# mrluin/TextualDegRemoval

Measured on AMD Instinct MI355X. Metric: train images/sec (512x512, bs=4/GPU), higher is better.
Workload: dtype f32 (3xbf16-split MFMA: 24-bit operand significands on the full fp32 exponent range, fp32 accumulate; unscaled gradients, no loss scale, no step-skip guard; tensors fp32 -- the MASA-encoder ResidualBlock activations / gradients as three bf16 planes whose sum IS the fp32 value, bit for bit)

## Files before the change

### include/tdr.h

```cpp
#ifndef TDR_H
#define TDR_H
#include <stdint.h>
#ifdef __cplusplus
extern "C" {
#endif

#define TDR_ABI_VERSION 112
int tdr_version(void);
const char* tdr_last_error(void);

typedef struct TdrStepGuard {
    float scale, inv_scale, max_scale;
    int good, growth_interval;
    int step, skipped, finite;
    float bc1, bc2_sqrt;
} TdrStepGuard;

typedef struct TdrConvDesc {
    int N, Cin, H, W;
    int Cout, OH, OW;
    int KH, stride, dil, pad;
    const float* in;  int64_t in_ns;
    int gate;
    const float* kscale; int64_t kscale_ns;
    const void* wp;  int64_t wp_ns;  int Mpad;
    int wp_fmt;
    float* out; int64_t out_ns;
    int epi;
    const float* bias;  int64_t bias_ns;
    const float* scale; int64_t scale_ns;
    const float* bias2; int64_t bias2_ns; float bias2_mul;
    const float* res;   int64_t res_ns;
    const float* mask;  int64_t mask_ns;
    const float* aux;   int64_t aux_ns;
    int relu;
} TdrConvDesc;

int tdr_conv_forward(const TdrConvDesc* d, void* stream);

int tdr_conv_ck(int KH_eff);
int64_t tdr_packed_weight_floats(int M, int Kch, int KH_eff);
int tdr_pack_weights(const float* w, int Cout, int Cin, int KH, int mode, float* wp, void* stream);
int64_t tdr_packed_weight_bytes_bx3(int M, int Kch, int KH_eff);
int tdr_pack_weights_bx3(const float* w, int Cout, int Cin, int KH, int mode, void* wp, void* stream);
int tdr_pack_weights_bx3_batch(const float* w, int64_t w_stride, int B, int Cout, int Cin, int KH, int mode, void* wp,
                               void* stream);
int64_t tdr_packed_weight_bytes_hx2(int M, int Kch, int KH_eff);
int tdr_pack_weights_hx2(const float* w, int Cout, int Cin, int KH, int mode, void* wp, void* stream);
int tdr_conv_force_cfg(int kh, int cfg);
typedef struct TdrPackJob {
    const float* w; void* wp;
    int Cout, Cin, KH, mode, fmt;
    int M, Kch, KHe, CK, Mx;
    int64_t total;
    int64_t first_block;
} TdrPackJob;
int tdr_pack_job_init(TdrPackJob* job, const float* w, int Cout, int Cin, int KH, int mode, int fmt, void* wp);
int tdr_pack_weights_multi(const TdrPackJob* jobs_dev, int n_jobs, int64_t total_blocks, void* stream);
int tdr_pack_patches(const float* blk, int B, int G, int C, int BH, int BW, int PH, int PW, int pstep, int dil,
                     int off, float* wp, void* stream);

typedef struct TdrConvP16Desc {
    int N, Cin, H, W, Cout;
    const void* in;
    const void* wp; int Mpad; int wp_fmt;
    const float* bias;
    const float* res32;  int64_t res32_ns;
    const void*  res16;
    const float* mask32; int64_t mask32_ns;
    const void*  mask16;
    int relu;
    float* out32; int64_t out32_ns;
    void*  out16;
} TdrConvP16Desc;
int64_t tdr_p16_bytes(int N, int C, int H, int W);
int tdr_p16_from_f32(const float* src, int64_t src_ns, int N, int C, int H, int W, void* dst, void* stream);
int tdr_p16_to_f32(const void* src, int N, int C, int H, int W, float* dst, int64_t dst_ns, void* stream);
int64_t tdr_p16_bytes_fmt(int N, int C, int H, int W, int fmt);
int tdr_p16_from_f32_fmt(const float* src, int64_t src_ns, int N, int C, int H, int W, void* dst, int fmt, void* stream);
int tdr_p16_to_f32_fmt(const void* src, int N, int C, int H, int W, float* dst, int64_t dst_ns, int fmt, void* stream);
int tdr_conv3x3_p16(const TdrConvP16Desc* d, void* stream);
int tdr_conv3x3_p16_force_cfg(int cfg);
// ... 458 lines not shown
```

### profiles/probe_conv1x1_deep.py

```python
import os, sys
sys.path.insert(0, os.path.dirname(os.path.dirname(os.path.abspath(__file__))))
import torch
from textualdegremoval_amd import kernels as K, _lib
K.set_math('bx3')
torch.manual_seed(0)
lib = _lib.load()


def t(N, Cin, Cout, H, mode):
    xs = [torch.randn(N, Cin, H, H, device='cuda') for _ in range(2)]
    w = torch.randn(Cout, Cin, 1, 1, device='cuda') * 0.05
    wp, mp, *_ = K.pack_weights(w, mode)
    co = Cout if mode == K.PACK_FWD else Cin
    xin = xs if mode == K.PACK_FWD else [torch.randn(N, Cout, H, H, device='cuda') for _ in range(2)]
    outs = [torch.empty(N, co, H, H, device='cuda') for _ in range(2)]
    line = f'1x1 {Cin}->{Cout} @{H} N{N} {"fwd  " if mode == K.PACK_FWD else "dgrad"}:'
    flop = 2.0 * N * Cin * Cout * H * H
    for cfg in (0, 1, 2, 3, 4, 5):
        lib.tdr_conv_force_cfg(1, cfg)
        f = lambda i: K.conv_forward(xin[i & 1], wp, mp, co, 1, pad=0, out=outs[i & 1])
        for i in range(3): f(i)
        torch.cuda.synchronize()
        g = torch.cuda.CUDAGraph()
        s = torch.cuda.Stream()
        with torch.cuda.stream(s):
            with torch.cuda.graph(g, stream=s):
                for i in range(20): f(i)
        g.replay(); torch.cuda.synchronize()
        e0, e1 = torch.cuda.Event(enable_timing=True), torch.cuda.Event(enable_timing=True)
        e0.record()
        for _ in range(5): g.replay()
        e1.record(); torch.cuda.synchronize()
        us = e0.elapsed_time(e1) / 100 * 1e3
        line += f'  c{cfg} {us:6.1f} us ({flop / us * 1e-6:4.0f} TF)'
    lib.tdr_conv_force_cfg(1, 0)
    print(line, flush=True)


for (Cin, Cout) in [(1024, 2048), (1024, 1024), (1024, 512), (512, 1024), (512, 512)]:
    t(4, Cin, Cout, 32, K.PACK_FWD)
    t(4, Cin, Cout, 32, K.PACK_DGRAD_S1)
```

### textualdegremoval_amd/_lib.py

```python
import ctypes as C
import os

import torch

_HERE = os.path.dirname(os.path.abspath(__file__))
LIB_PATH = os.environ.get('TDR_LIB_PATH', os.path.join(_HERE, 'libtdr_hip.so'))

ABI_VERSION = 112
c_fp = C.c_void_p
i32, i64, f32 = C.c_int, C.c_int64, C.c_float


class TdrConvDesc(C.Structure):
    _fields_ = [
        ('N', i32), ('Cin', i32), ('H', i32), ('W', i32),
        ('Cout', i32), ('OH', i32), ('OW', i32),
        ('KH', i32), ('stride', i32), ('dil', i32), ('pad', i32),
        ('inp', c_fp), ('in_ns', i64),
        ('gate', i32),
        ('kscale', c_fp), ('kscale_ns', i64),
        ('wp', c_fp), ('wp_ns', i64), ('Mpad', i32), ('wp_fmt', i32),
        ('out', c_fp), ('out_ns', i64),
        ('epi', i32),
        ('bias', c_fp), ('bias_ns', i64),
# ... 165 lines not shown
    'tdr_dwsg_fwd': (i32, [c_fp, c_fp, c_fp, i32, i32, i32, i32, c_fp, c_fp, c_fp, c_fp]),
    'tdr_dwsg_bwd': (i32, [c_fp, c_fp, c_fp, c_fp, i32, i32, i32, i32, c_fp, c_fp, c_fp, c_fp, c_fp]),
    'tdr_dwsg_bwd_biased': (i32, [c_fp, c_fp, f32, c_fp, c_fp, c_fp, i32, i32, i32, i32, c_fp, c_fp, c_fp, c_fp, c_fp]),
    'tdr_dwsg_bwd_parts_supported': (i32, [i32]),
    'tdr_dw_param_finish': (i32, [c_fp, i32, i32, i32, i32, c_fp, c_fp, c_fp]),
    'tdr_dwgelu_fwd': (i32, [c_fp, c_fp, c_fp, i32, i32, i32, i32, c_fp, c_fp]),
    'tdr_dwgelu_bwd': (i32, [c_fp, c_fp, c_fp, c_fp, i32, i32, i32, i32, c_fp, c_fp, c_fp, c_fp, c_fp]),
    'tdr_dwconv_fwd': (i32, [c_fp, c_fp, c_fp, i32, i32, i32, i32, c_fp, c_fp]),
    'tdr_dwconv_act_fwd': (i32, [c_fp, c_fp, c_fp, i32, i32, i32, i32, i32, c_fp, c_fp]),
    'tdr_dwconv_act_bwd': (i32, [c_fp, c_fp, c_fp, c_fp, i32, i32, i32, i32, c_fp, c_fp, c_fp, c_fp, c_fp]),
    'tdr_dwpair_fwd': (i32, [c_fp, c_fp, c_fp, i32, i32, i32, i32, i32, c_fp, i64, c_fp]),
    'tdr_dwpair_bwd': (i32, [c_fp, i64, c_fp, i64, c_fp, c_fp, i32, i32, i32, i32, c_fp, c_fp, c_fp, c_fp, c_fp]),
    'tdr_dwconv_halves_fwd': (i32, [c_fp, c_fp, c_fp, i32, i32, i32, i32, i32, c_fp, c_fp, i64, c_fp]),
    'tdr_dwconv_halves_bwd': (i32, [c_fp, c_fp, i64, c_fp, c_fp, i64, c_fp, c_fp, i32, i32, i32, i32, c_fp, c_fp, c_fp, c_fp, c_fp]),
    'tdr_dwconv_bwd': (i32, [c_fp, c_fp, c_fp, i32, i32, i32, i32, c_fp, c_fp, c_fp, c_fp, c_fp]),
    'tdr_row_sumsq': (i32, [c_fp, i64, i32, i32, i32, c_fp, c_fp]),
    'tdr_mdta_pad': (i32, [i32]),
    'tdr_mdta_softmax': (i32, [c_fp, c_fp, c_fp, i32, i32, i32, c_fp, c_fp, c_fp]),
    'tdr_mdta_bwd': (i32, [c_fp, c_fp, c_fp, c_fp, c_fp, i32, i32, i32, c_fp, c_fp, c_fp, c_fp]),
    'tdr_attn_fold_proj': (i32, [c_fp, c_fp, i32, i32, i32, c_fp, c_fp]),
    'tdr_axpby_dev': (i32, [c_fp, c_fp, c_fp, i64, c_fp, c_fp]),
    'tdr_dot': (i32, [c_fp, c_fp, i64, c_fp, c_fp, c_fp]),
    'tdr_pixel_shuffle2': (i32, [c_fp, i32, i32, i32, i32, c_fp, c_fp]),
    'tdr_leaky_relu_fwd': (i32, [c_fp, i64, f32, c_fp, c_fp]),
    'tdr_leaky_relu_bwd': (i32, [c_fp, c_fp, i64, f32, c_fp, c_fp]),
    'tdr_gather_col': (i32, [c_fp, i32, i32, i32, i32, c_fp, c_fp]),
    'tdr_mapper_combine': (i32, [c_fp, c_fp, i32, i32, i32, i32, i32, i32, c_fp, c_fp]),
    'tdr_mapper_combine_bwd': (i32, [c_fp, i32, i32, i32, i32, i32, i32, c_fp, c_fp, c_fp]),
    'tdr_cross_attention_fwd': (i32, [c_fp, c_fp, c_fp, i32, i32, i32, i32, i32, i32, i32, f32, c_fp, c_fp, c_fp]),
    'tdr_cross_attention_bwd': (i32, [c_fp, c_fp, c_fp, c_fp, c_fp, c_fp, i32, i32, i32, i32, i32, i32, i32, f32, c_fp, c_fp,
                                      c_fp, c_fp, c_fp]),
    'tdr_transpose_pad': (i32, [c_fp, i32, i32, i32, i32, c_fp, c_fp]),
    'tdr_conv_force_cfg': (i32, [i32, i32]),
    'tdr_packed_weight_bytes_hx2': (i64, [i32, i32, i32]),
    'tdr_pack_weights_hx2': (i32, [c_fp, i32, i32, i32, i32, c_fp, c_fp]),
    'tdr_pack_weights_bx3_batch': (i32, [c_fp, i64, i32, i32, i32, i32, i32, c_fp, c_fp]),
    'tdr_sca_fwd': (i32, [c_fp, c_fp, c_fp, i32, i32, c_fp, c_fp]),
    'tdr_sca_bwd': (i32, [c_fp] * 8 + [i32, i32] + [c_fp] * 7 + [c_fp]),
    'tdr_gelu_fwd': (i32, [c_fp, c_fp, i32, i32, c_fp, c_fp, i64, c_fp]),
    'tdr_gelu_bwd': (i32, [c_fp, c_fp, c_fp, i64, c_fp]),
    'tdr_subsample2': (i32, [c_fp, i32, i32, i32, c_fp, c_fp]),
    'tdr_instnorm_fwd': (i32, [c_fp, c_fp, c_fp, f32, i32, i32, i32, c_fp, c_fp, c_fp, c_fp]),
    'tdr_instnorm_bwd': (i32, [c_fp] * 5 + [i32, i32, i32] + [c_fp] * 5),
    'tdr_region_affine_fwd': (i32, [c_fp, i64, c_fp, c_fp, f32, i32, i32, i32, i32, i32, c_fp, i64, c_fp, c_fp]),
    'tdr_region_affine_bwd': (i32, [c_fp, i64, c_fp, i64, c_fp, c_fp, f32, c_fp, i32, i32, i32, i32, i32, c_fp, i64, c_fp, c_fp, c_fp, c_fp]),
    'tdr_sf_dyn_vec_fwd': (i32, [C.POINTER(TdrSfDynVecDesc), c_fp]),
    'tdr_sf_dyn_vec_bwd': (i32, [C.POINTER(TdrSfDynVecBwdDesc), c_fp]),
    'tdr_sf_dynfilt_fwd': (i32, [c_fp, i64, c_fp, c_fp, c_fp, i32, i32, i32, i32, i32, i32, c_fp, c_fp, c_fp]),
    'tdr_sf_dynfilt_bwd_reduce': (i32, [c_fp, c_fp, i64, c_fp, c_fp, c_fp, i32, i32, i32, i32, i32, i32, c_fp, c_fp, c_fp, c_fp]),
    'tdr_sf_dynfilt_bwd_dx': (i32, [c_fp] * 5 + [i32] * 6 + [c_fp, i64, c_fp]),
    'tdr_convt4_weight_to_3x3': (i32, [c_fp, c_fp, i32, i32, c_fp, c_fp, c_fp]),
    'tdr_convt4_grad_from_3x3': (i32, [c_fp, c_fp, i32, i32, c_fp, c_fp, c_fp]),
    'tdr_sf_region_split': (i32, [c_fp, i64, i32, i32, i32, i32, i32, c_fp, c_fp]),
    'tdr_sf_local_affine': (i32, [c_fp, i64, c_fp, c_fp, c_fp, f32, i32, i32, i32, i32, i32, c_fp, i64, c_fp]),
    'tdr_sf_emerge': (i32, [c_fp, i64, c_fp, i32, i32, i32, c_fp, c_fp]),
    'tdr_sf_softmax_mix': (i32, [c_fp, i64, c_fp, c_fp, c_fp, i32, i32, i32, c_fp, c_fp]),
    'tdr_scaled_conv_param_grads': (i32, [c_fp] * 5 + [i32, i32] + [c_fp] * 3 + [c_fp]),
    'tdr_pair_sum_partials_multi': (i32, [c_fp, i32, i32, c_fp]),
    'tdr_dw_param_finish_nb': (i32, [i32, i32]),
    'tdr_dw_param_finish_multi': (i32, [c_fp, i32, i32, c_fp]),
    'tdr_scaled_conv_param_grads_multi': (i32, [c_fp, i32, i32, c_fp]),
    'tdr_chansum_ws_floats': (i64, [i32, i32, i32]),
    'tdr_channel_sum': (i32, [c_fp, i64, i32, i32, i32, c_fp, c_fp, c_fp]),
    'tdr_copy_rows': (i32, [c_fp, i64, c_fp, i64, i32, i64, c_fp]),
    'tdr_add_rows': (i32, [c_fp, i64, c_fp, i64, i32, i64, c_fp]),
    'tdr_pixel_unshuffle2': (i32, [c_fp, i32, i32, i32, i32, c_fp, c_fp]),
# ... 152 lines not shown
```

### textualdegremoval_amd/csrc/tdr_conv_bx3.hip

```cpp
#include <stdlib.h>
#include "tdr_common.h"
#include "tdr_conv_epi.h"
#include "tdr_pack.h"
#include "../../include/tdr.h"

typedef __bf16 bf16x8 __attribute__((ext_vector_type(8)));


namespace {

constexpr int bx_cmax(int a, int b) { return a > b ? a : b; }
constexpr int bx_plane(int NT, int TW, int KH, int S) {
    return (((NT * 32 / TW) - 1) * S + KH) * ((TW - 1) * S + KH);
}
constexpr int bx_max_plane(int NT, int KH, int S) {
    return bx_cmax(bx_plane(NT, 8, KH, S), bx_cmax(bx_plane(NT, 16, KH, S), bx_plane(NT, 32, KH, S)));
}

__device__ __forceinline__ void split3(float x, __bf16& h, __bf16& m, __bf16& l) {
    h = (__bf16)x;
    const float r = x - (float)h;
    m = (__bf16)r;
    l = (__bf16)(r - (float)m);
}
// ... 414 lines not shown
    if constexpr (EPI != EPI_PSHUF) {
        if (a.vec_epi) {
            conv_epilogue_vec<TM, TN, EPI>(a, acc, n, m0, wm, wn, oy0, ox0, lane, reinterpret_cast<float*>(smem4) + wave * (32 * 36));
            return;
        }
    }
    conv_epilogue<TM, TN, EPI>(a, acc, n, m0, wm, wn, oy0, ox0, j, kk);
}

template <int WM, int TM, int TN, int EPI, bool GATE, int SCH>
int launch_c1_hx2(const ConvArgs& a, int N, hipStream_t st) {
    constexpr int WN = 4 / WM;
    constexpr int BM = 32 * TM * WM;
    constexpr int NT = TN * WN;
    const int TW = 1 << a.tw_log2, SR = 32 >> a.tw_log2, TH = NT * SR;
    ConvArgs b = a;
    b.tiles_x = tdr_cdiv(a.OW, TW);
    const int tiles_y = tdr_cdiv(a.OH, TH);
    b.mtiles = tdr_cdiv(a.Cout, BM);
    dim3 grid(b.tiles_x * tiles_y * b.mtiles, 1, N);
    b.single_buf = 0;
    const size_t lds = 2 * 32768;
    auto kern = conv1x1_hx2_kernel<WM, TM, TN, EPI, GATE, SCH>;
    static bool attr_set = false;
    if (!attr_set) {
        (void)hipFuncSetAttribute(reinterpret_cast<const void*>(kern), hipFuncAttributeMaxDynamicSharedMemorySize, 160 * 1024);
        attr_set = true;
    }
    hipLaunchKernelGGL(kern, grid, dim3(256), lds, st, b);
    TDR_LAUNCH_CHECK("conv1x1_hx2_kernel");
    return TDR_OK;
}

inline bool c1_hx2_ok(const ConvArgs& a, int npx, int bm, int N) {
    static const bool off = tdr_tune_env("TDR_C1_OLD") != nullptr;
    static const int min_stages = tdr_tune_env("TDR_C1_STAGES") ? atoi(tdr_tune_env("TDR_C1_STAGES")) : 4;
    static const long max_blocks = tdr_tune_env("TDR_C1_BLOCKS") ? atol(tdr_tune_env("TDR_C1_BLOCKS")) : 512;
    const int ks = 8192 / npx;
    const long blocks = (long)tdr_cdiv((long)a.OH * a.OW, npx) * tdr_cdiv(a.Cout, bm) * N;
    return !off && blocks <= max_blocks && (a.Cin + ks - 1) / ks >= min_stages && a.pad == 0 && a.W % 4 == 0 && a.in_ns % 4 == 0 && (reinterpret_cast<uintptr_t>(a.in) & 15) == 0 &&
           a.H == a.OH && a.W == a.OW;
}

template <int KH, int S, int WM, int TM, int TN, int EPI, bool GATE, int SCH>
int launch_bx_cfg_s(const ConvArgs& a, int N, hipStream_t st) {
    if constexpr (KH == 1 && S == 1 && SCH != SCH_BX3 && EPI != EPI_PSHUF)
        if (c1_hx2_ok(a, 32 * TN * (4 / WM), 32 * TM * WM, N)) return launch_c1_hx2<WM, TM, TN, EPI, GATE, SCH>(a, N, st);
    constexpr int NS = SCH == SCH_BX3 ? 3 : (SCH == SCH_HX2 ? 2 : 1);
    constexpr int WN = 4 / WM;
    constexpr int BM = 32 * TM * WM;
    constexpr int NT = TN * WN;
    const int TW = 1 << a.tw_log2, SR = 32 >> a.tw_log2, TH = NT * SR;
    const int LH = (TH - 1) * S + KH, LW = (TW - 1) * S + KH;
    ConvArgs b = a;
    static const int single_env = tdr_tune_env("TDR_BX_SINGLE") ? atoi(tdr_tune_env("TDR_BX_SINGLE")) : 2;
    b.single_buf = (KH == 3 && (a.Cin + 15) / 16 <= single_env) ? 1 : 0;
    size_t lds = (size_t)(b.single_buf ? 1 : 2) * (2 * NS) * LH * LW * 16;
    if (lds < 4 * 32 * 36 * sizeof(float)) lds = 4 * 32 * 36 * sizeof(float);
    b.tiles_x = tdr_cdiv(a.OW, TW);
    const int tiles_y = tdr_cdiv(a.OH, TH);
    b.mtiles = tdr_cdiv(a.Cout, BM);
    dim3 grid(b.tiles_x * tiles_y * b.mtiles, 1, N);
    if constexpr (KH == 3 && S == 1 && SCH == SCH_HX2 && EPI == EPI_STD && !GATE) {
        static const int ring3 = tdr_tune_env("TDR_RING3") ? atoi(tdr_tune_env("TDR_RING3")) : 1;
        static const long ring_blocks3 = tdr_tune_env("TDR_RING_BLOCKS") ? atol(tdr_tune_env("TDR_RING_BLOCKS")) : 512;
        if (ring3 && ((long)grid.x * N > ring_blocks3 || TM != 1)) {
            auto kern = conv_bx3_kernel<KH, S, WM, TM, TN, EPI, GATE, SCH, 3>;
            static bool attr_set = false;
            if (!attr_set) {
                (void)hipFuncSetAttribute(reinterpret_cast<const void*>(kern), hipFuncAttributeMaxDynamicSharedMemorySize, 160 * 1024);
                attr_set = true;
            }
            hipLaunchKernelGGL(kern, grid, dim3(256), lds, st, b);
            TDR_LAUNCH_CHECK("conv_bx3_kernel(ring3)");
            return TDR_OK;
        }
    }
    if constexpr (KH == 3 && S == 1 && TM == 1 && SCH == SCH_HX2 && EPI == EPI_STD) {
        static const long ring_blocks = tdr_tune_env("TDR_RING_BLOCKS") ? atol(tdr_tune_env("TDR_RING_BLOCKS")) : 512;
        if ((long)grid.x * N <= ring_blocks) {
            auto kern = conv_bx3_kernel<KH, S, WM, TM, TN, EPI, GATE, SCH, 9>;
            static bool attr_set = false;
            if (!attr_set) {
                (void)hipFuncSetAttribute(reinterpret_cast<const void*>(kern), hipFuncAttributeMaxDynamicSharedMemorySize, 160 * 1024);
                attr_set = true;
            }
            hipLaunchKernelGGL(kern, grid, dim3(256), lds, st, b);
            TDR_LAUNCH_CHECK("conv_bx3_kernel(ring)");
            return TDR_OK;
        }
    }
    auto kern = conv_bx3_kernel<KH, S, WM, TM, TN, EPI, GATE, SCH>;
    static bool attr_set = false;
    if (!attr_set) {
        (void)hipFuncSetAttribute(reinterpret_cast<const void*>(kern), hipFuncAttributeMaxDynamicSharedMemorySize, 160 * 1024);
        attr_set = true;
    }
    hipLaunchKernelGGL(kern, grid, dim3(256), lds, st, b);
    TDR_LAUNCH_CHECK("conv_bx3_kernel");
    return TDR_OK;
}

int g_force_cfg[2] = {tdr_tune_env("TDR_BX_CFG1") ? atoi(tdr_tune_env("TDR_BX_CFG1")) : 0, tdr_tune_env("TDR_BX_CFG3") ? atoi(tdr_tune_env("TDR_BX_CFG3")) : 0};

template <int KH, int S, int WM, int TM, int TN, int EPI, bool GATE>
int launch_bx_cfg(const ConvArgs& a, int N, hipStream_t st) {
    if (a.scheme == SCH_HX2) return launch_bx_cfg_s<KH, S, WM, TM, TN, EPI, GATE, SCH_HX2>(a, N, st);
    if (a.scheme == SCH_H1) return launch_bx_cfg_s<KH, S, WM, TM, TN, EPI, GATE, SCH_H1>(a, N, st);
    return launch_bx_cfg_s<KH, S, WM, TM, TN, EPI, GATE, SCH_BX3>(a, N, st);
}

template <int KH, int S, int EPI, bool GATE>
int launch_bx_shape(const ConvArgs& a, int N, hipStream_t st) {
    const long pix = (long)a.OH * a.OW;
    auto blocks = [&](int bm, int bn) { return (long)tdr_cdiv(a.Cout, bm) * tdr_cdiv(pix, bn) * N; };
    if constexpr (S == 2) {
        if (a.Cout <= 32) return launch_bx_cfg<KH, S, 1, 1, 1, EPI, GATE>(a, N, st);
        if (a.Cout <= 64 || blocks(128, 64) < 512) return launch_bx_cfg<KH, S, 2, 1, 1, EPI, GATE>(a, N, st);
        return launch_bx_cfg<KH, S, 2, 2, 1, EPI, GATE>(a, N, st);
    } else {
        if (a.Cout <= 32) {
            if (blocks(32, 256) >= 512) return launch_bx_cfg<KH, S, 1, 1, 2, EPI, GATE>(a, N, st);
            return launch_bx_cfg<KH, S, 1, 1, 1, EPI, GATE>(a, N, st);
        }
        if (g_force_cfg[KH == 1 ? 0 : 1] == 0 && a.scheme == SCH_BX3 && a.Cin <= (KH == 1 ? 128 : 64) && blocks(64, 128) >= 2048)
            return launch_bx_cfg<KH, S, 2, 1, 2, EPI, GATE>(a, N, st);
        if constexpr (KH == 1) {
            const int force = g_force_cfg[0];
            if (force == 1) return launch_bx_cfg<KH, S, 2, 2, 2, EPI, GATE>(a, N, st);
            if (force == 2) return launch_bx_cfg<KH, S, 2, 1, 4, EPI, GATE>(a, N, st);
            if (force == 3) return launch_bx_cfg<KH, S, 2, 1, 2, EPI, GATE>(a, N, st);
            if (force == 4) return launch_bx_cfg<KH, S, 1, 1, 2, EPI, GATE>(a, N, st);
            if (force == 5) return launch_bx_cfg<KH, S, 4, 2, 2, EPI, GATE>(a, N, st);
            if (a.Cout > 64 && blocks(128, 128) >= 512) return launch_bx_cfg<KH, S, 2, 2, 2, EPI, GATE>(a, N, st);
            if (a.Cin >= 768 && a.Cout >= 256 && blocks(256, 64) >= 256 && blocks(256, 64) <= 512)
                return launch_bx_cfg<KH, S, 4, 2, 2, EPI, GATE>(a, N, st);
        } else {
            const int force3 = g_force_cfg[1];
            if (force3 == 1) return launch_bx_cfg<KH, S, 2, 2, 4, EPI, GATE>(a, N, st);
            if (force3 == 2) return launch_bx_cfg<KH, S, 2, 1, 4, EPI, GATE>(a, N, st);
            if (force3 == 3) return launch_bx_cfg<KH, S, 2, 1, 2, EPI, GATE>(a, N, st);
            if (force3 == 4) return launch_bx_cfg<KH, S, 2, 2, 2, EPI, GATE>(a, N, st);
            const bool tall_ok = blocks(128, 256) >= 1024 || a.Cout % 128 != 0 || a.scheme != SCH_HX2;
            if (a.Cout > 64 && blocks(128, 256) >= 512 && tall_ok) return launch_bx_cfg<KH, S, 2, 2, 4, EPI, GATE>(a, N, st);
        }
        if (blocks(64, 256) >= 512) return launch_bx_cfg<KH, S, 2, 1, 4, EPI, GATE>(a, N, st);
        return launch_bx_cfg<KH, S, 2, 1, 2, EPI, GATE>(a, N, st);
    }
}

__global__ void pack_weights_bx3_kernel(const float* __restrict__ w, long w_bs, int Cout, int Cin, int KH, int mode, int M,
                                        int Kch, int KHe, int MT, long total, uint4* __restrict__ wp, long wp_bs16) {
    const float* wb = w + (long)blockIdx.y * w_bs;
    uint4* ob = wp + (long)blockIdx.y * wp_bs16;
    for (long i = blockIdx.x * (long)blockDim.x + threadIdx.x; i < total; i += (long)gridDim.x * blockDim.x)
        tdr_pack_bx3_frag(wb, Cin, KH, mode, M, Kch, KHe, MT, i, ob);
}

__global__ void pack_weights_hx2_kernel(const float* __restrict__ w, int Cout, int Cin, int KH, int mode, int M, int Kch, int KHe,
                                        int MT, long total, uint4* __restrict__ wp) {
    for (long i = blockIdx.x * (long)blockDim.x + threadIdx.x; i < total; i += (long)gridDim.x * blockDim.x)
        tdr_pack_hx2_frag(w, Cin, KH, mode, M, Kch, KHe, MT, i, wp);
}

}

extern "C" int tdr_conv_force_cfg(int kh, int cfg) {
    g_force_cfg[kh == 1 ? 0 : 1] = cfg;
    return TDR_OK;
}

extern "C" int64_t tdr_packed_weight_bytes_bx3(int M, int Kch, int KH_eff) {
    const long MT = (M + 31) / 32;
    return (long)((Kch + 15) / 16) * KH_eff * KH_eff * MT * 3 * 1024;
}

extern "C" int tdr_pack_weights_bx3(const float* w, int Cout, int Cin, int KH, int mode, void* wp, void* stream) {
    TDR_REQUIRE(w && wp, "tdr_pack_weights_bx3: null pointer");
    TDR_REQUIRE(mode >= 0 && mode <= 3, "tdr_pack_weights_bx3: bad mode %d", mode);
    int M, Kch, KHe;
    if (mode == 0) { M = Cout; Kch = Cin; KHe = KH; }
    else if (mode == 1) { M = Cin; Kch = Cout; KHe = KH; }
    else if (mode == 2) { TDR_REQUIRE(KH == 2, "mode 2 needs a 2x2 kernel"); M = 4 * Cin; Kch = Cout; KHe = 1; }
    else { TDR_REQUIRE(KH == 3, "mode 3 needs a 3x3 kernel"); M = 4 * Cin; Kch = Cout; KHe = 2; }
    const int MT = (M + 31) / 32;
    const long total = (long)((Kch + 15) / 16) * KHe * KHe * MT * 64;
    const int blocks = (int)((total + 255) / 256 < 4096 ? (total + 255) / 256 : 4096);
    hipLaunchKernelGGL(pack_weights_bx3_kernel, dim3(blocks), dim3(256), 0, (hipStream_t)stream, w, 0L, Cout, Cin, KH, mode, M,
                       Kch, KHe, MT, total, (uint4*)wp, 0L);
    TDR_LAUNCH_CHECK("pack_weights_bx3_kernel");
    return TDR_OK;
}

extern "C" int64_t tdr_packed_weight_bytes_hx2(int M, int Kch, int KH_eff) {
    const long MT = (M + 31) / 32;
    return (long)((Kch + 15) / 16) * KH_eff * KH_eff * MT * 2 * 1024;
}

extern "C" int tdr_pack_weights_hx2(const float* w, int Cout, int Cin, int KH, int mode, void* wp, void* stream) {
    TDR_REQUIRE(w && wp, "tdr_pack_weights_hx2: null pointer");
    TDR_REQUIRE(mode >= 0 && mode <= 3, "tdr_pack_weights_hx2: bad mode %d", mode);
    int M, Kch, KHe;
// ... 66 lines not shown
```

### textualdegremoval_amd/kernels.py

```python
import contextlib
import ctypes as C
import os

import torch

from . import _lib
from ._lib import TdrConvDesc, TdrConvP16Desc, TdrWgradDesc, TdrWgradP16Desc, check

EPI_STD, EPI_GATEBWD, EPI_PSHUF = 0, 1, 2
PACK_FWD, PACK_DGRAD_S1, PACK_DGRAD_2X2S2, PACK_DGRAD_3X3S2 = 0, 1, 2, 3

MATH = os.environ.get('TDR_MATH', 'bx3')
WGRAD_1X1_BX3 = True
FMT_F32, FMT_BX3, FMT_HX2, FMT_H1 = 0, 1, 2, 3


def fp16_path():
    return MATH in ('hx2', 'h1')


GRAD_SCALED = False
BACKWARD_PHASE = False


# ... 35 lines not shown
        per = x[0].numel()
        ns = x.stride(0) if n > 1 else per
        assert x[0].is_contiguous()
        check(_lib.load().tdr_absmax_bits(x.data_ptr(), ns, n, per, self.table.data_ptr() + 4 * i, _stream()), 'tdr_absmax_bits')

    def read(self):
        bits = self.table[:len(self.kinds)].cpu().numpy().astype('int64') & 0xffffffff
        out = {}
        for kind in ('fwd', 'grad'):
            b = [int(v) for v, k in zip(bits, self.kinds) if k == kind and v != 0]
            bad = sum(1 for v in b if v >= 0x7f800000)
            e = [((v >> 23) & 0xff) - 127 for v in b if v < 0x7f800000]
            out[kind] = (min(e), max(e), bad) if e else (None, None, bad)
        return out


_survey = None


class PackedWeights:
    __slots__ = ('buf', 'fmt')

    def __init__(self, buf, fmt):
        self.buf, self.fmt = buf, fmt

    def data_ptr(self):
        return self.buf.data_ptr()


ATTN_F32 = False
ATTN_BX3 = True
DWK_GENERIC = False
SIDE_WGRAD = False
_side_stream = None
_side_active = False
_side_dirty = False
_side_keep = []


class on_side:
    def __init__(self, *keep):
        self.keep = keep
        self.on = False

    def __enter__(self):
        global _side_stream, _side_active, _side_dirty
        if SIDE_WGRAD and not _side_active:
            if _side_stream is None:
                _side_stream = torch.cuda.Stream()
            _side_stream.wait_stream(torch.cuda.current_stream())
            _side_active = _side_dirty = self.on = True
            _side_keep.extend(self.keep)
        return self

    def __exit__(self, *exc):
        global _side_active
        if self.on:
            _side_active = False
        return False


def side_keep(*tensors):
    if _side_active:
        _side_keep.extend(tensors)
    return tensors[0] if len(tensors) == 1 else tensors

# ... 240 lines not shown
    if e is None:
        w4 = [W[g].view(Cout, Cin, 1, 1) for g in range(G)]
        proto = _packed_buffer(w4[0], mode, MATH)
        per = proto.buf.numel()
        big = torch.empty(G * per, dtype=torch.float32, device=W.device)
        views = [PackedWeights(big[g * per:(g + 1) * per], proto.fmt) for g in range(G)]
        for g in range(G):
            _pack_into(w4[g], mode, views[g])
            if plan is not None:
                plan.entries[(w4[g].data_ptr(), tuple(w4[g].shape), mode, MATH, GRAD_SCALED)] = (w4[g], mode, MATH, views[g])
        M = _pack_dims(w4[0], mode)[0]
        e = (PackedWeights(big, proto.fmt), (M + 31) // 32 * 32, per, w4, views)
        if plan is not None:
            plan.dirty = True
            store[key] = e
    elif not plan.valid:
        for w, v in zip(e[3], e[4]):
            _pack_into(w, mode, v)
    return e[0], e[1], e[2]


def pack_patches(blk, G, PH, PW, pstep, dil, off):
    lib = _lib.load()
    BG, Cc, BH, BW = blk.shape
    B = BG // G
    M = G * PH * PW
    per_b = lib.tdr_packed_weight_floats(M, Cc, 3)
    wp = torch.empty(B * per_b, dtype=torch.float32, device=blk.device)
    check(lib.tdr_pack_patches(blk.data_ptr(), B, G, Cc, BH, BW, PH, PW, pstep, dil, off, wp.data_ptr(), _stream()),
          'tdr_pack_patches')
    return wp, (M + 31) // 32 * 32, per_b


def conv_forward(x, wp, Mpad, Cout, KH, stride=1, dil=1, pad=0, OH=None, OW=None, out=None, Cin=None, epi=EPI_STD,
                 gate=False, kscale=None, wp_ns=0, bias=None, scale=None, bias2=None, bias2_mul=1.0, res=None,
                 mask=None, aux=None, relu=False):
    lib = _lib.load()
    N, Cx, H, W = x.shape
    if Cin is None:
        Cin = Cx // 2 if gate else Cx
    if OH is None:
        OH = (H + 2 * pad - dil * (KH - 1) - 1) // stride + 1
        OW = (W + 2 * pad - dil * (KH - 1) - 1) // stride + 1
    if out is None:
        if epi == EPI_PSHUF:
            out = torch.empty(N, Cout // 4, 2 * OH, 2 * OW, dtype=torch.float32, device=x.device)
        elif epi == EPI_GATEBWD:
            out = torch.empty(N, 2 * Cout, OH, OW, dtype=torch.float32, device=x.device)
        else:
            out = torch.empty(N, Cout, OH, OW, dtype=torch.float32, device=x.device)
    d = TdrConvDesc()
    d.N, d.Cin, d.H, d.W = N, Cin, H, W
    d.Cout, d.OH, d.OW = Cout, OH, OW
    d.KH, d.stride, d.dil, d.pad = KH, stride, dil, pad
    d.inp, d.in_ns = x.data_ptr(), _dense_nchw(x)
    d.gate = 1 if gate else 0
    d.kscale, d.kscale_ns = _p(kscale), _vec_ns(kscale)
    d.wp, d.wp_ns, d.Mpad = wp.data_ptr(), wp_ns, Mpad
    d.wp_fmt = getattr(wp, 'fmt', FMT_F32)
    d.out, d.out_ns = out.data_ptr(), _dense_nchw(out)
    d.epi = epi
    d.bias, d.bias_ns = _p(bias), _vec_ns(bias)
    d.scale, d.scale_ns = _p(scale), _vec_ns(scale)
    d.bias2, d.bias2_ns, d.bias2_mul = _p(bias2), _vec_ns(bias2), float(bias2_mul)
    d.res, d.res_ns = _p(res), (_dense_nchw(res) if res is not None else 0)
    d.mask, d.mask_ns = _p(mask), (_dense_nchw(mask) if mask is not None else 0)
    d.aux, d.aux_ns = _p(aux), (_dense_nchw(aux) if aux is not None else 0)
    d.relu = int(relu) if not isinstance(relu, bool) else (1 if relu else 0)
    if _survey is not None and d.wp_fmt in (FMT_HX2, FMT_H1):
        _survey.probe(x, 'grad' if BACKWARD_PHASE else 'fwd')
    check(lib.tdr_conv_forward(C.byref(d), _stream()), 'tdr_conv_forward')
    return out


class P16:
    __slots__ = ('buf', 'N', 'C', 'H', 'W', 'fmt')

    def __init__(self, buf, N, Cc, H, W, fmt=FMT_HX2):
        self.buf, self.N, self.C, self.H, self.W, self.fmt = buf, N, Cc, H, W, fmt

    @staticmethod
    def empty(N, Cc, H, W, device, fmt=FMT_HX2):
        assert Cc % 16 == 0, f'plane tensors need C % 16 == 0 (got {Cc})'
        assert fmt in (FMT_HX2, FMT_BX3)
        n = _lib.load().tdr_p16_bytes_fmt(N, Cc, H, W, fmt) // 4
        return P16(torch.empty(n, dtype=torch.int32, device=device), N, Cc, H, W, fmt)

    def data_ptr(self):
        return self.buf.data_ptr()

    def to_f32(self):
        out = torch.empty(self.N, self.C, self.H, self.W, dtype=torch.float32, device=self.buf.device)
        check(_lib.load().tdr_p16_to_f32_fmt(self.buf.data_ptr(), self.N, self.C, self.H, self.W, out.data_ptr(), _dense_nchw(out),
                                             self.fmt, _stream()), 'tdr_p16_to_f32')
        return out


def p16_supported(Cc):
    return Cc % 16 == 0 and Cc >= 16


def plane_fmt():
    if MATH == 'hx2' and GRAD_SCALED:
        return FMT_HX2
    if MATH == 'bx3':
# ... 1866 lines not shown
```

Measured before the change: 60.97.

## Add staged register-prefetch 1x1 bx3 conv kernel with wide loads

Adds a new 1x1 stride-1 bx3 convolution kernel. It loads several input channels per thread as float4 into registers two stages ahead, splits them into three bf16 planes, and writes them into double-buffered 24 KiB LDS stages, so there is one barrier per stage rather than per 16-channel group. The kernel is enabled by default when the shape qualifies: no padding, W divisible by 4, aligned input and at least four stages. Python toggles and a query path are added for probing. The cost is higher register pressure and LDS use per block, which may lower occupancy.

```diff
diff --git a/include/tdr.h b/include/tdr.h
--- a/include/tdr.h
+++ b/include/tdr.h
@@ -48,6 +48,8 @@
 int64_t tdr_packed_weight_bytes_hx2(int M, int Kch, int KH_eff);
 int tdr_pack_weights_hx2(const float* w, int Cout, int Cin, int KH, int mode, void* wp, void* stream);
 int tdr_conv_force_cfg(int kh, int cfg);
+int tdr_conv1x1_bx3_staged_set(int on);
+int tdr_conv1x1_bx3_staged_takes(const TdrConvDesc* d);
 typedef struct TdrPackJob {
     const float* w; void* wp;
     int Cout, Cin, KH, mode, fmt;
diff --git a/profiles/probe_conv1x1_deep.py b/profiles/probe_conv1x1_deep.py
--- a/profiles/probe_conv1x1_deep.py
+++ b/profiles/probe_conv1x1_deep.py
@@ -16,8 +16,10 @@
     outs = [torch.empty(N, co, H, H, device='cuda') for _ in range(2)]
     line = f'1x1 {Cin}->{Cout} @{H} N{N} {"fwd  " if mode == K.PACK_FWD else "dgrad"}:'
     flop = 2.0 * N * Cin * Cout * H * H
-    for cfg in (0, 1, 2, 3, 4, 5):
-        lib.tdr_conv_force_cfg(1, cfg)
+    for cfg in (-1, 0, 1, 2, 3, 4, 5):
+        K.CONV1X1_STAGED = cfg != -1
+        lib.tdr_conv_force_cfg(1, max(cfg, 0))
+        staged = K.conv1x1_staged_takes(xin[0], wp, mp, co, 1, pad=0, out=outs[0])
         f = lambda i: K.conv_forward(xin[i & 1], wp, mp, co, 1, pad=0, out=outs[i & 1])
         for i in range(3): f(i)
         torch.cuda.synchronize()
@@ -32,7 +34,7 @@
         for _ in range(5): g.replay()
         e1.record(); torch.cuda.synchronize()
         us = e0.elapsed_time(e1) / 100 * 1e3
-        line += f'  c{cfg} {us:6.1f} us ({flop / us * 1e-6:4.0f} TF)'
+        line += f'  {"g0" if cfg < 0 else f"c{cfg}"}{"s" if staged else " "} {us:6.1f} us ({flop / us * 1e-6:4.0f} TF)'
     lib.tdr_conv_force_cfg(1, 0)
     print(line, flush=True)
 
diff --git a/profiles/probe_conv1x1_staged_cap.py b/profiles/probe_conv1x1_staged_cap.py
--- /dev/null
+++ b/profiles/probe_conv1x1_staged_cap.py
@@ -0,0 +1,39 @@
+import os, sys
+sys.path.insert(0, os.path.dirname(os.path.dirname(os.path.abspath(__file__))))
+import torch
+from textualdegremoval_amd import kernels as K
+K.set_math('bx3')
+torch.manual_seed(0)
+
+
+def t(N, Cin, Cout, H):
+    xs = [torch.randn(N, Cin, H, H, device='cuda') for _ in range(2)]
+    wp, mp, *_ = K.pack_weights(torch.randn(Cout, Cin, 1, 1, device='cuda') * 0.05, K.PACK_FWD)
+    outs = [torch.empty(N, Cout, H, H, device='cuda') for _ in range(2)]
+    line = f'1x1 {Cin}->{Cout} @{H} N{N}:'
+    for on in (False, True):
+        K.CONV1X1_STAGED = on
+        staged = K.conv1x1_staged_takes(xs[0], wp, mp, Cout, 1, out=outs[0])
+        f = lambda i: K.conv_forward(xs[i & 1], wp, mp, Cout, 1, out=outs[i & 1])
+        for i in range(3): f(i)
+        torch.cuda.synchronize()
+        g = torch.cuda.CUDAGraph()
+        s = torch.cuda.Stream()
+        with torch.cuda.stream(s):
+            with torch.cuda.graph(g, stream=s):
+                for i in range(20): f(i)
+        g.replay(); torch.cuda.synchronize()
+        e0, e1 = torch.cuda.Event(enable_timing=True), torch.cuda.Event(enable_timing=True)
+        e0.record()
+        for _ in range(5): g.replay()
+        e1.record(); torch.cuda.synchronize()
+        line += f'  {"staged " if staged else "generic"} {e0.elapsed_time(e1) / 100 * 1e3:6.1f} us'
+    K.CONV1X1_STAGED = True
+    print(line, flush=True)
+
+
+for (Cin, Cout, H) in [(512, 1024, 64), (1024, 512, 64), (512, 512, 64), (256, 512, 128), (256, 256, 128), (128, 256, 256)]:
+    t(4, Cin, Cout, H)
+print('256-pixel tiles (16-channel stages: one barrier per 16 channels as in the generic kernel, only the load width differs):', flush=True)
+for (N, Cin, Cout, H) in [(8, 64, 32, 256), (8, 256, 32, 128), (8, 256, 64, 128), (8, 512, 64, 128), (4, 64, 32, 512)]:
+    t(N, Cin, Cout, H)
diff --git a/textualdegremoval_amd/_lib.py b/textualdegremoval_amd/_lib.py
--- a/textualdegremoval_amd/_lib.py
+++ b/textualdegremoval_amd/_lib.py
@@ -221,6 +221,8 @@
                                       c_fp, c_fp, c_fp]),
     'tdr_transpose_pad': (i32, [c_fp, i32, i32, i32, i32, c_fp, c_fp]),
     'tdr_conv_force_cfg': (i32, [i32, i32]),
+    'tdr_conv1x1_bx3_staged_set': (i32, [i32]),
+    'tdr_conv1x1_bx3_staged_takes': (i32, [C.POINTER(TdrConvDesc)]),
     'tdr_packed_weight_bytes_hx2': (i64, [i32, i32, i32]),
     'tdr_pack_weights_hx2': (i32, [c_fp, i32, i32, i32, i32, c_fp, c_fp]),
     'tdr_pack_weights_bx3_batch': (i32, [c_fp, i64, i32, i32, i32, i32, i32, c_fp, c_fp]),
diff --git a/textualdegremoval_amd/csrc/tdr_conv_bx3.hip b/textualdegremoval_amd/csrc/tdr_conv_bx3.hip
--- a/textualdegremoval_amd/csrc/tdr_conv_bx3.hip
+++ b/textualdegremoval_amd/csrc/tdr_conv_bx3.hip
@@ -470,6 +470,179 @@
     return TDR_OK;
 }
 
+template <int WM, int TM, int TN, int EPI, bool GATE>
+__global__ __launch_bounds__(256, 2) void conv1x1_bx3s_kernel(ConvArgs a) {
+    constexpr int NS = 3, NP = 6;
+    constexpr int WN = 4 / WM;
+    constexpr int BM = 32 * TM * WM;
+    constexpr int NT = TN * WN;
+    constexpr int NPX = 32 * NT;
+    constexpr int QUADS = NPX / 4;
+    constexpr int HOCT = 256 / QUADS;
+    constexpr int KS = 4 * HOCT;
+    constexpr int OCT = KS / 8;
+    constexpr int GPS = KS / 16;
+    constexpr int PFD = 2;
+    static_assert(GPS >= 1 && NS * OCT * NPX * 16 == 24576, "a stage is 24 KiB");
+
+    extern __shared__ __attribute__((aligned(16))) uint4 smem4[];
+
+    const int tid = threadIdx.x, lane = tid & 63, wave = __builtin_amdgcn_readfirstlane(tid >> 6);
+    const int wm = wave / WN, wn = wave % WN;
+    const int j = lane & 31, kk = lane >> 5;
+    const int TW = 1 << a.tw_log2, SR = 32 >> a.tw_log2, TH = NT * SR;
+    int logical;
+    {
+        const int T = gridDim.x, b = blockIdx.x;
+        const int q = T >> 3, r = T & 7, xcd = b & 7, slot = b >> 3;
+        logical = (xcd < r ? xcd * (q + 1) : r * (q + 1) + (xcd - r) * q) + slot;
+    }
+    const int mtile = logical % a.mtiles, ptile = logical / a.mtiles;
+    const int tx = ptile % a.tiles_x, ty = ptile / a.tiles_x;
+    const int m0 = mtile * BM;
+    const int n = blockIdx.z;
+    const int oy0 = ty * TH, ox0 = tx * TW;
+    const long HWin = (long)a.H * a.W;
+
+    const int sh = tid / QUADS, sq = tid % QUADS;
+    const int p0 = 4 * sq;
+    const int gy = oy0 + (p0 >> a.tw_log2), gx = ox0 + (p0 & (TW - 1));
+    const bool pok = gy < a.H && gx < a.W;
+    const long goff = pok ? (long)gy * a.W + gx : 0;
+    const float* in_n = a.in + (long)n * a.in_ns;
+    const float* ks_n = a.kscale ? a.kscale + (long)n * a.kscale_ns : nullptr;
+    const int ngroups = (a.Cin + 15) >> 4;
+    const int nstages = (a.Cin + KS - 1) / KS;
+
+    float4 rin[PFD][4];
+    float4 rin2[GATE ? PFD : 1][GATE ? 4 : 1];
+    float rks[PFD][4];
+    auto load_stage = [&](int st, int set) {
+        const int cbase = st * KS + sh * 4;
+#pragma unroll
+        for (int i = 0; i < 4; ++i) {
+            const int ci = cbase + i;
+            rin[set][i] = make_float4(0.f, 0.f, 0.f, 0.f);
+            rks[set][i] = 1.f;
+            if (GATE) rin2[set][i] = make_float4(0.f, 0.f, 0.f, 0.f);
+            if (pok && ci < a.Cin) {
+                const float* src = in_n + (long)ci * HWin + goff;
+                rin[set][i] = *reinterpret_cast<const float4*>(src);
+                if (GATE) rin2[set][i] = *reinterpret_cast<const float4*>(src + a.gate_off);
+                if (ks_n) rks[set][i] = ks_n[ci];
+            }
+        }
+    };
+    int wslot[4];
+#pragma unroll
+    for (int i = 0; i < 4; ++i) wslot[i] = 2 * ((sh >> 1) * NPX + swz1(p0 + i)) + (sh & 1);
+    auto store_stage = [&](int set, int buf) {
+        uint2* sb = reinterpret_cast<uint2*>(smem4 + buf * (NS * OCT * NPX));
+#pragma unroll
+        for (int px = 0; px < 4; ++px) {
+            union { uint2 u; __bf16 v[4]; } h, m, l;
+#pragma unroll
+            for (int i = 0; i < 4; ++i) {
+                const float4 q4 = rin[set][i];
+                float v = px == 0 ? q4.x : (px == 1 ? q4.y : (px == 2 ? q4.z : q4.w));
+                if (GATE) {
+                    const float4 g4 = rin2[set][i];
+                    v *= px == 0 ? g4.x : (px == 1 ? g4.y : (px == 2 ? g4.z : g4.w));
+                }
+                v *= rks[set][i];
+                asm volatile("" : "+v"(v));
+                __bf16 hh, mm, ll;
+                split3(v, hh, mm, ll);
+                h.v[i] = hh; m.v[i] = mm; l.v[i] = ll;
+            }
+            sb[wslot[px]] = h.u;
+            sb[2 * (OCT * NPX) + wslot[px]] = m.u;
+            sb[4 * (OCT * NPX) + wslot[px]] = l.u;
+        }
+    };
+
+    int bslot[TN];
+#pragma unroll
+    for (int tn = 0; tn < TN; ++tn) bslot[tn] = kk * NPX + swz1(32 * (wn * TN + tn) + j);
+    const int MT = a.Mpad >> 5;
+    const uint4* wfrag[TM];
+#pragma unroll
+    for (int tm = 0; tm < TM; ++tm) {
+        const int mt = min((m0 >> 5) + wm * TM + tm, MT - 1);
+        wfrag[tm] = reinterpret_cast<const uint4*>(a.wp) + (long)n * (a.wp_ns >> 2) + (long)mt * (NS * 64) + lane;
+    }
+    const long wstep = (long)MT * (NS * 64);
+
+    f32x16 acc[TM][TN];
+#pragma unroll
+    for (int tm = 0; tm < TM; ++tm)
+#pragma unroll
+        for (int tn = 0; tn < TN; ++tn)
+#pragma unroll
+            for (int r = 0; r < 16; ++r) acc[tm][tn][r] = 0.f;
+
+    Frag af[TM][NS], afn[TM][NS];
+    auto load_a = [&](Frag (&dst)[TM][NS], long g) {
+#pragma unroll
+        for (int tm = 0; tm < TM; ++tm)
+#pragma unroll
+            for (int s = 0; s < NS; ++s) dst[tm][s].u = wfrag[tm][g * wstep + s * 64];
+    };
+
+    load_a(af, 0);
+#pragma unroll
+    for (int p = 0; p < PFD; ++p)
+        if (p < nstages) load_stage(p, p);
+    store_stage(0, 0);
+    __syncthreads();
+
+    for (int s0 = 0; s0 < nstages; s0 += PFD) {
+#pragma unroll
+        for (int u = 0; u < PFD; ++u) {
+            const int st = s0 + u;
+            if (st < nstages) {
+                const int buf = st & 1;
+                const uint4* sb = smem4 + buf * (NS * OCT * NPX);
+#pragma unroll
+                for (int gg = 0; gg < GPS; ++gg) {
+                    const int g = st * GPS + gg;
+                    if (g < ngroups) {
+                        load_a(afn, min(g + 1, ngroups - 1));
+                        if (gg == 0 && st + PFD < nstages) load_stage(st + PFD, u);
+                        Frag bf[TN][NS];
+#pragma unroll
+                        for (int tn = 0; tn < TN; ++tn)
+#pragma unroll
+                            for (int s = 0; s < NS; ++s) bf[tn][s].u = sb[s * (OCT * NPX) + 2 * gg * NPX + bslot[tn]];
+                        constexpr int SA[6] = {2, 0, 1, 1, 0, 0}, SB[6] = {0, 2, 1, 0, 1, 0};
+#pragma unroll
+                        for (int q = 0; q < NP; ++q)
+#pragma unroll
+                            for (int tm = 0; tm < TM; ++tm)
+#pragma unroll
+                                for (int tn = 0; tn < TN; ++tn)
+                                    acc[tm][tn] = __builtin_amdgcn_mfma_f32_32x32x16_bf16(af[tm][SA[q]].v, bf[tn][SB[q]].v, acc[tm][tn], 0, 0, 0);
+#pragma unroll
+                        for (int tm = 0; tm < TM; ++tm)
+#pragma unroll
+                            for (int s = 0; s < NS; ++s) af[tm][s] = afn[tm][s];
+                    }
+                }
+                if (st + 1 < nstages) store_stage((u + 1) % PFD, buf ^ 1);
+                __syncthreads();
+            }
+        }
+    }
+
+    if constexpr (EPI != EPI_PSHUF) {
+        if (a.vec_epi) {
+            conv_epilogue_vec<TM, TN, EPI>(a, acc, n, m0, wm, wn, oy0, ox0, lane, reinterpret_cast<float*>(smem4) + wave * (32 * 36));
+            return;
+        }
+    }
+    conv_epilogue<TM, TN, EPI>(a, acc, n, m0, wm, wn, oy0, ox0, j, kk);
+}
+
 inline bool c1_hx2_ok(const ConvArgs& a, int npx, int bm, int N) {
     static const bool off = tdr_tune_env("TDR_C1_OLD") != nullptr;
     static const int min_stages = tdr_tune_env("TDR_C1_STAGES") ? atoi(tdr_tune_env("TDR_C1_STAGES")) : 4;
@@ -480,8 +653,44 @@
            a.H == a.OH && a.W == a.OW;
 }
 
+template <int WM, int TM, int TN, int EPI, bool GATE>
+int launch_c1_bx3s(const ConvArgs& a, int N, hipStream_t st) {
+    constexpr int WN = 4 / WM;
+    constexpr int BM = 32 * TM * WM;
+    constexpr int NT = TN * WN;
+    const int TW = 1 << a.tw_log2, SR = 32 >> a.tw_log2, TH = NT * SR;
+    ConvArgs b = a;
+    b.tiles_x = tdr_cdiv(a.OW, TW);
+    const int tiles_y = tdr_cdiv(a.OH, TH);
+    b.mtiles = tdr_cdiv(a.Cout, BM);
+    dim3 grid(b.tiles_x * tiles_y * b.mtiles, 1, N);
+    b.single_buf = 0;
+    const size_t lds = 2 * 24576;
+    hipLaunchKernelGGL((conv1x1_bx3s_kernel<WM, TM, TN, EPI, GATE>), grid, dim3(256), lds, st, b);
+    TDR_LAUNCH_CHECK("conv1x1_bx3s_kernel");
+    return TDR_OK;
+}
+
+int g_force_cfg[2] = {tdr_tune_env("TDR_BX_CFG1") ? atoi(tdr_tune_env("TDR_BX_CFG1")) : 0, tdr_tune_env("TDR_BX_CFG3") ? atoi(tdr_tune_env("TDR_BX_CFG3")) : 0};
+int g_c1_bx3_staged = 1;
+thread_local int* g_c1_bx3_query = nullptr;
+
+inline bool c1_bx3_ok(const ConvArgs& a, int npx, int bm, int N) {
+    static const long max_blocks = tdr_tune_env("TDR_C1_BLOCKS") ? atol(tdr_tune_env("TDR_C1_BLOCKS")) : (1L << 40);
+    const int ks = 4096 / npx;
+    const long blocks = (long)tdr_cdiv((long)a.OH * a.OW, npx) * tdr_cdiv(a.Cout, bm) * N;
+    return g_c1_bx3_staged && g_force_cfg[0] == 0 && blocks <= max_blocks && (a.Cin + ks - 1) / ks >= 4 && a.pad == 0 && a.W % 4 == 0 && a.in_ns % 4 == 0 &&
+           (reinterpret_cast<uintptr_t>(a.in) & 15) == 0 && a.H == a.OH && a.W == a.OW;
+}
+
 template <int KH, int S, int WM, int TM, int TN, int EPI, bool GATE, int SCH>
 int launch_bx_cfg_s(const ConvArgs& a, int N, hipStream_t st) {
+    if constexpr (KH == 1 && S == 1 && SCH == SCH_BX3 && EPI != EPI_PSHUF) {
+        const bool staged = c1_bx3_ok(a, 32 * TN * (4 / WM), 32 * TM * WM, N);
+        if (g_c1_bx3_query) { *g_c1_bx3_query = staged ? 1 : 0; return TDR_OK; }
+        if (staged) return launch_c1_bx3s<WM, TM, TN, EPI, GATE>(a, N, st);
+    }
+    if (g_c1_bx3_query) return TDR_OK;
     if constexpr (KH == 1 && S == 1 && SCH != SCH_BX3 && EPI != EPI_PSHUF)
         if (c1_hx2_ok(a, 32 * TN * (4 / WM), 32 * TM * WM, N)) return launch_c1_hx2<WM, TM, TN, EPI, GATE, SCH>(a, N, st);
     constexpr int NS = SCH == SCH_BX3 ? 3 : (SCH == SCH_HX2 ? 2 : 1);
@@ -539,8 +748,6 @@
     return TDR_OK;
 }
 
-int g_force_cfg[2] = {tdr_tune_env("TDR_BX_CFG1") ? atoi(tdr_tune_env("TDR_BX_CFG1")) : 0, tdr_tune_env("TDR_BX_CFG3") ? atoi(tdr_tune_env("TDR_BX_CFG3")) : 0};
-
 template <int KH, int S, int WM, int TM, int TN, int EPI, bool GATE>
 int launch_bx_cfg(const ConvArgs& a, int N, hipStream_t st) {
     if (a.scheme == SCH_HX2) return launch_bx_cfg_s<KH, S, WM, TM, TN, EPI, GATE, SCH_HX2>(a, N, st);
@@ -606,6 +813,20 @@
 extern "C" int tdr_conv_force_cfg(int kh, int cfg) {
     g_force_cfg[kh == 1 ? 0 : 1] = cfg;
     return TDR_OK;
+}
+
+extern "C" int tdr_conv1x1_bx3_staged_set(int on) {
+    g_c1_bx3_staged = on ? 1 : 0;
+    return TDR_OK;
+}
+
+extern "C" int tdr_conv1x1_bx3_staged_takes(const TdrConvDesc* d) {
+    if (!d || d->wp_fmt != 1 || d->dil != 1 || d->KH != 1 || d->stride != 1) return 0;
+    int takes = 0;
+    g_c1_bx3_query = &takes;
+    const int rc = tdr_conv_forward(d, nullptr);
+    g_c1_bx3_query = nullptr;
+    return rc == TDR_OK ? takes : 0;
 }
 
 extern "C" int64_t tdr_packed_weight_bytes_bx3(int M, int Kch, int KH_eff) {
diff --git a/textualdegremoval_amd/kernels.py b/textualdegremoval_amd/kernels.py
--- a/textualdegremoval_amd/kernels.py
+++ b/textualdegremoval_amd/kernels.py
@@ -91,6 +91,8 @@
 ATTN_BX3 = True
 DWK_GENERIC = False
 SIDE_WGRAD = False
+CONV1X1_STAGED = True
+_conv1x1_staged_sent = True
 _side_stream = None
 _side_active = False
 _side_dirty = False
@@ -397,10 +399,9 @@
     return wp, (M + 31) // 32 * 32, per_b
 
 
-def conv_forward(x, wp, Mpad, Cout, KH, stride=1, dil=1, pad=0, OH=None, OW=None, out=None, Cin=None, epi=EPI_STD,
-                 gate=False, kscale=None, wp_ns=0, bias=None, scale=None, bias2=None, bias2_mul=1.0, res=None,
-                 mask=None, aux=None, relu=False):
-    lib = _lib.load()
+def _conv_desc(x, wp, Mpad, Cout, KH, stride=1, dil=1, pad=0, OH=None, OW=None, out=None, Cin=None, epi=EPI_STD,
+               gate=False, kscale=None, wp_ns=0, bias=None, scale=None, bias2=None, bias2_mul=1.0, res=None,
+               mask=None, aux=None, relu=False):
     N, Cx, H, W = x.shape
     if Cin is None:
         Cin = Cx // 2 if gate else Cx
@@ -432,10 +433,34 @@
     d.mask, d.mask_ns = _p(mask), (_dense_nchw(mask) if mask is not None else 0)
     d.aux, d.aux_ns = _p(aux), (_dense_nchw(aux) if aux is not None else 0)
     d.relu = int(relu) if not isinstance(relu, bool) else (1 if relu else 0)
+    return d, out
+
+
+def _sync_conv1x1_staged(lib):
+    global _conv1x1_staged_sent
+    if bool(CONV1X1_STAGED) != _conv1x1_staged_sent:
+        check(lib.tdr_conv1x1_bx3_staged_set(1 if CONV1X1_STAGED else 0), 'tdr_conv1x1_bx3_staged_set')
+        _conv1x1_staged_sent = bool(CONV1X1_STAGED)
+
+
+def conv_forward(x, wp, Mpad, Cout, KH, stride=1, dil=1, pad=0, OH=None, OW=None, out=None, Cin=None, epi=EPI_STD,
+                 gate=False, kscale=None, wp_ns=0, bias=None, scale=None, bias2=None, bias2_mul=1.0, res=None,
+                 mask=None, aux=None, relu=False):
+    lib = _lib.load()
+    d, out = _conv_desc(x, wp, Mpad, Cout, KH, stride, dil, pad, OH, OW, out, Cin, epi, gate, kscale, wp_ns, bias, scale, bias2,
+                        bias2_mul, res, mask, aux, relu)
     if _survey is not None and d.wp_fmt in (FMT_HX2, FMT_H1):
         _survey.probe(x, 'grad' if BACKWARD_PHASE else 'fwd')
+    _sync_conv1x1_staged(lib)
     check(lib.tdr_conv_forward(C.byref(d), _stream()), 'tdr_conv_forward')
     return out
+
+
+def conv1x1_staged_takes(x, wp, Mpad, Cout, KH, *args, **kw):
+    lib = _lib.load()
+    d, _ = _conv_desc(x, wp, Mpad, Cout, KH, *args, **kw)
+    _sync_conv1x1_staged(lib)
+    return bool(lib.tdr_conv1x1_bx3_staged_takes(C.byref(d)))
 
 
 class P16:
```

After: 61.86 (median of 6 runs). 1.01x the previous value.
